# jynik/OOKiedokie

Measured on AMD Instinct MI355X. Metric: IQ Msamples/s demodulated (SC16Q11->bits), higher is better.
Workload: dtype f32

## Files before the change

### ookiedokie_amd/csrc/fir_mfma.hip

```cpp
#include "kernels.hpp"
#include "common.hpp"

#include <hip/hip_ext.h>

#include <algorithm>
#include <cmath>
#include <cstring>
#include <type_traits>

#pragma clang fp contract(off)

namespace ookd {

typedef _Float16 h8 __attribute__((ext_vector_type(8)));
typedef _Float16 h4 __attribute__((ext_vector_type(4)));
typedef float f16x __attribute__((ext_vector_type(16)));
typedef float v2fm __attribute__((ext_vector_type(2)));
typedef short v2s __attribute__((ext_vector_type(2)));
typedef uint32_t v4u __attribute__((ext_vector_type(4)));

__host__ __device__ constexpr uint32_t mslot(uint32_t j) { return j + 8u * (j >> 5); }

template <int KS, int FMT = (int)kFmtSc16>
struct MfmaGeom {
    static constexpr uint32_t Tp = 16u * (KS - 2);
    static constexpr uint32_t W = kMfmaTile + Tp;
    static constexpr uint32_t plane = mslot(W);
    static constexpr uint32_t lds_bytes = plane * 2u * 2u;
    static constexpr uint32_t vsamples = FMT == (int)kFmtSc16 ? 4u : 8u;
    static constexpr uint32_t nvec = W / vsamples;
    static constexpr int rounds = (int)((nvec + 63u) / 64u);
};

typedef const __attribute__((address_space(1))) v4u *gptr128;
__device__ __forceinline__ uint4 ld_nt4m(gptr128 p) {
    const v4u v = __builtin_nontemporal_load(p);
    return make_uint4(v.x, v.y, v.z, v.w);
}

typedef const __attribute__((address_space(1))) unsigned char *gbytes;
typedef __attribute__((address_space(1))) unsigned char *gbytes_w;
__device__ __forceinline__ uint4 ld_nt4_at(gbytes base, uint32_t byte_off) {
    const v4u v = __builtin_nontemporal_load(reinterpret_cast<gptr128>(base + byte_off));
    return make_uint4(v.x, v.y, v.z, v.w);
}

template <typename P>
__device__ __forceinline__ P uniform_ptr(P ptr) {
    uint64_t v = (uint64_t)ptr;
    asm volatile("" : "+s"(v));
    return (P)v;
}

__device__ __forceinline__ v2s as_v2sm(uint32_t w) { return __builtin_bit_cast(v2s, w); }

typedef const __attribute__((address_space(1))) uint32_t *gptr32;
typedef const __attribute__((address_space(1))) uint16_t *gptr16;
typedef const __attribute__((address_space(1))) float *gptrf;

template <int FMT>
struct RawSrcT {
    typedef typename std::conditional<FMT == (int)kFmtSc16, uint32_t, uint16_t>::type elem;
    typedef const __attribute__((address_space(1))) elem *ptr;
    ptr src;
    ptr halo;
    uint32_t halo_len;
    uint64_t n_valid;
};

typedef RawSrcT<(int)kFmtSc16> RawSrc;

template <int FMT>
__device__ __forceinline__ uint32_t fetch_fmt_m(const RawSrcT<FMT> &rs, int64_t n) {
    const uint32_t z = FMT == (int)kFmtSc16 ? 0u : zero8<FMT>();
    if (n < 0) {
        const int64_t h = (int64_t)rs.halo_len + n;
        if (h < 0 || !rs.halo) return z;
        return rs.halo[h];
    }
    if ((uint64_t)n >= rs.n_valid) return z;
    return rs.src[n];
}

template <int FMT>
__device__ __forceinline__ uint32_t fetch_raw_m(const RawSrcT<FMT> &rs, int64_t n) {
    if (n < 0) {
        const int64_t h = (int64_t)rs.halo_len + n;
        if (h < 0 || !rs.halo) return 0u;
        if constexpr (FMT == (int)kFmtSc16) return rs.halo[h];
        else return widen8<FMT>(rs.halo[h]);
    }
    if ((uint64_t)n >= rs.n_valid) return 0u;
    if constexpr (FMT == (int)kFmtSc16) return rs.src[n];
    else return widen8<FMT>(rs.src[n]);
}

template <int FMT>
__device__ __forceinline__ float2 mfma_exact_output(const RawSrcT<FMT> &rs, gptrf taps, uint32_t T, int64_t n) {
    const float s = 1.0f / 2048.0f;
    float re = 0.0f, im = 0.0f;
    for (uint32_t k = 0; k < T; ++k) {
        const uint32_t w = fetch_raw_m(rs, n - (int64_t)k);
        const float xr = (float)(int16_t)(w & 0xffffu) * s;
        const float xi = (float)(int16_t)(w >> 16) * s;
        const float t = taps[k];
        const float pr = t * xr;
        const float pi = t * xi;
        re = re + pr;
        im = im + pi;
    }
    return make_float2(re, im);
}

template <int HALF>
__device__ __forceinline__ uint32_t cvt2(uint32_t a, uint32_t b) {
    uint32_t r;
    if (HALF == 0) {
        asm("v_cvt_f16_i16_sdwa %0, %1 dst_sel:WORD_0 dst_unused:UNUSED_PAD src0_sel:WORD_0" : "=v"(r) : "v"(a));
        asm("v_cvt_f16_i16_sdwa %0, %1 dst_sel:WORD_1 dst_unused:UNUSED_PRESERVE src0_sel:WORD_0" : "+v"(r) : "v"(b));
    } else {
        asm("v_cvt_f16_i16_sdwa %0, %1 dst_sel:WORD_0 dst_unused:UNUSED_PAD src0_sel:WORD_1" : "=v"(r) : "v"(a));
        asm("v_cvt_f16_i16_sdwa %0, %1 dst_sel:WORD_1 dst_unused:UNUSED_PRESERVE src0_sel:WORD_1" : "+v"(r) : "v"(b));
    }
    return r;
}

__device__ __forceinline__ void cvt4(uint4 q, uint32_t mask, uint2 &re, uint2 &im) {
    const uint32_t w0 = q.x & mask, w1 = q.y & mask, w2 = q.z & mask, w3 = q.w & mask;
    re = make_uint2(cvt2<0>(w0, w1), cvt2<0>(w2, w3));
    im = make_uint2(cvt2<1>(w0, w1), cvt2<1>(w2, w3));
}

typedef _Float16 h2 __attribute__((ext_vector_type(2)));
typedef unsigned short v2us __attribute__((ext_vector_type(2)));

template <int FMT>
__device__ __forceinline__ void expand8(uint32_t w, uint32_t &re, uint32_t &im) {
    if (FMT == (int)kFmtCs8) w ^= 0x80808080u;
    re = __builtin_amdgcn_perm(0x64646464u, w, 0x04020400u);
    im = __builtin_amdgcn_perm(0x64646464u, w, 0x04030401u);
}

__device__ __forceinline__ uint32_t scale8(uint32_t t) {
    const h2 k = {(_Float16)16.0f, (_Float16)16.0f}, b = {(_Float16)-18432.0f, (_Float16)-18432.0f};
    return __builtin_bit_cast(uint32_t, __builtin_elementwise_fma(__builtin_bit_cast(h2, t), k, b));
}

template <int FMT>
__device__ __forceinline__ void cvt8(uint4 q, uint4 &re, uint4 &im) {
    uint32_t r0, r1, r2, r3, i0, i1, i2, i3;
    expand8<FMT>(q.x, r0, i0);
    expand8<FMT>(q.y, r1, i1);
    expand8<FMT>(q.z, r2, i2);
    expand8<FMT>(q.w, r3, i3);
    re = make_uint4(scale8(r0), scale8(r1), scale8(r2), scale8(r3));
    im = make_uint4(scale8(i0), scale8(i1), scale8(i2), scale8(i3));
}

template <int FMT, int ROUNDS>
__device__ __forceinline__ void window_levels8(const uint4 (&q)[ROUNDS], int L, bool &loud) {
    v2us mx = (v2us){0x6480, 0x6480}, mn = mx;
#pragma unroll
    for (int i = 0; i < ROUNDS; ++i) {
        const uint32_t w[4] = {q[i].x, q[i].y, q[i].z, q[i].w};
#pragma unroll
        for (int k = 0; k < 4; ++k) {
            uint32_t re, im;
            expand8<FMT>(w[k], re, im);
            const v2us a = __builtin_bit_cast(v2us, re), b = __builtin_bit_cast(v2us, im);
            mx = __builtin_elementwise_max(mx, __builtin_elementwise_max(a, b));
            mn = __builtin_elementwise_min(mn, __builtin_elementwise_min(a, b));
        }
    }
    const int m = (L - 1) >> 4;
    const uint32_t hi = 0x6480u + (uint32_t)(m < 127 ? m : 127), lo = 0x6480u - (uint32_t)(m < 128 ? m : 128);
    loud = L <= 0 || mx.x > hi || mx.y > hi || mn.x < lo || mn.y < lo;
}

template <int KS>
__host__ __device__ constexpr int mfma_waves() { return KS <= 6 ? 4 : KS <= 10 ? 8 : 16; }
constexpr uint32_t kMfmaCtlBytes = 16;

template <int KS>
__host__ __device__ constexpr uint32_t mfma_lds_bytes() {
    return (uint32_t)KS * 2u * 1024u + kMfmaCtlBytes + (uint32_t)mfma_waves<KS>() * MfmaGeom<KS>::lds_bytes;
}

template <int FMT>
struct MfmaTileCtxT {
    RawSrcT<FMT> rs;
    uint32_t *ctl;
    uint32_t tickets;
    uint64_t tile_base, tile_end;
    uint32_t xcd_span;
    bool aligned16;
};

template <int FMT>
__device__ __forceinline__ bool mfma_take_ticket(const MfmaTileCtxT<FMT> &c, uint32_t tid, uint64_t &tile) {
    uint32_t tk = 0;
    if (tid == 0) tk = __hip_atomic_fetch_add(&c.ctl[0], 1u, __ATOMIC_RELAXED, __HIP_MEMORY_SCOPE_WORKGROUP);
    tk = (uint32_t)__builtin_amdgcn_readfirstlane((int)tk);
    const uint64_t v = (uint64_t)tk * gridDim.x + blockIdx.x;
    tile = (c.xcd_span ? (v & 7u) * (uint64_t)c.xcd_span + (v >> 3) : v) + c.tile_base;
    return tk < c.tickets && v + c.tile_base < c.tile_end;
}

template <int KS, int FMT>
__device__ __forceinline__ bool mfma_interior(const MfmaTileCtxT<FMT> &c, uint64_t tile) {
    const uint64_t t0 = tile * kMfmaTile;
    return c.aligned16 && t0 >= MfmaGeom<KS>::Tp && t0 + kMfmaTile <= c.rs.n_valid;
}

template <int KS, int FMT>
__device__ __forceinline__ void mfma_issue_loads(const MfmaTileCtxT<FMT> &c, uint64_t tile, uint32_t tid,
                                                 uint4 (&q)[MfmaGeom<KS, FMT>::rounds]) {
    using Gm = MfmaGeom<KS, FMT>;
    const gbytes src4 = uniform_ptr((gbytes)(c.rs.src + (tile * kMfmaTile - Gm::Tp)));
#pragma unroll
    for (int i = 0; i < Gm::rounds; ++i) {
        const uint32_t v = tid + 64u * i;
        q[i] = ld_nt4_at(src4, 16u * ((64u * (i + 1) <= Gm::nvec || v < Gm::nvec) ? v : Gm::nvec - 1u));
    }
}

template <int FMT>
__device__ __forceinline__ uint4 fetch_vec_m(const RawSrcT<FMT> &rs, int64_t s0) {
    uint4 w;
    if constexpr (FMT == (int)kFmtSc16) {
        w.x = fetch_raw_m(rs, s0);
        w.y = fetch_raw_m(rs, s0 + 1);
        w.z = fetch_raw_m(rs, s0 + 2);
        w.w = fetch_raw_m(rs, s0 + 3);
    } else {
        w.x = fetch_fmt_m(rs, s0) | (fetch_fmt_m(rs, s0 + 1) << 16);
        w.y = fetch_fmt_m(rs, s0 + 2) | (fetch_fmt_m(rs, s0 + 3) << 16);
        w.z = fetch_fmt_m(rs, s0 + 4) | (fetch_fmt_m(rs, s0 + 5) << 16);
        w.w = fetch_fmt_m(rs, s0 + 6) | (fetch_fmt_m(rs, s0 + 7) << 16);
    }
    return w;
}

template <int KS, int FMT>
__device__ __noinline__ void mfma_boundary_stage(RawSrcT<FMT> rs, uint64_t t0, uint32_t tid, uint4 *stage) {
    using Gm = MfmaGeom<KS, FMT>;
    for (uint32_t v = tid; v < Gm::nvec; v += 64u) {
        const int64_t s0 = (int64_t)t0 - (int64_t)Gm::Tp + (int64_t)Gm::vsamples * (int64_t)v;
        stage[v] = fetch_vec_m(rs, s0);
    }
}

template <int KS, int FMT>
__device__ __forceinline__ void mfma_boundary_loads(const MfmaTileCtxT<FMT> &c, uint64_t tile, uint32_t tid, unsigned char *win,
                                                    uint4 (&q)[MfmaGeom<KS, FMT>::rounds]) {
    using Gm = MfmaGeom<KS, FMT>;
    uint4 *stage = reinterpret_cast<uint4 *>(win);
    mfma_boundary_stage<KS, FMT>(c.rs, tile * kMfmaTile, tid, stage);
    __builtin_amdgcn_fence(__ATOMIC_RELEASE, "wavefront");
    __builtin_amdgcn_wave_barrier();
    __builtin_amdgcn_fence(__ATOMIC_ACQUIRE, "wavefront");
#pragma unroll
    for (int i = 0; i < Gm::rounds; ++i) {
        const uint32_t v = tid + 64u * i;
        q[i] = stage[(64u * (i + 1) <= Gm::nvec || v < Gm::nvec) ? v : Gm::nvec - 1u];
    }
    __builtin_amdgcn_fence(__ATOMIC_RELEASE, "wavefront");
    __builtin_amdgcn_wave_barrier();
}

template <int KS, int FMT>
__device__ __forceinline__ void mfma_convert(const uint4 (&q)[MfmaGeom<KS, FMT>::rounds], uint32_t mask, uint32_t tid,
                                             _Float16 *pl_re, _Float16 *pl_im) {
    using Gm = MfmaGeom<KS, FMT>;
#pragma unroll
    for (int i = 0; i < Gm::rounds; ++i) {
        const uint32_t v = tid + 64u * i;
        if (64u * (i + 1) <= Gm::nvec || v < Gm::nvec) {
            if constexpr (FMT == (int)kFmtSc16) {
                uint2 r4, i4;
                cvt4(q[i], mask, r4, i4);
                *reinterpret_cast<uint2 *>(pl_re + mslot(4u * v)) = r4;
                *reinterpret_cast<uint2 *>(pl_im + mslot(4u * v)) = i4;
            } else {
                uint4 r8, i8;
                cvt8<FMT>(q[i], r8, i8);
                *reinterpret_cast<uint4 *>(pl_re + mslot(8u * v)) = r8;
                *reinterpret_cast<uint4 *>(pl_im + mslot(8u * v)) = i8;
            }
        }
    }
    __builtin_amdgcn_fence(__ATOMIC_RELEASE, "wavefront");
    __builtin_amdgcn_wave_barrier();
    __builtin_amdgcn_fence(__ATOMIC_ACQUIRE, "wavefront");
}

template <int KS, bool FIRST>
__device__ __forceinline__ void mfma_ksteps(const h8 *a_img, const _Float16 *pl_re, const _Float16 *pl_im, uint32_t tid,
                                            f16x &are, f16x &aim) {
    const uint32_t n = tid & 31u, hh = tid >> 5;
    const _Float16 *bre = pl_re + 40u * n + 8u * hh;
    const _Float16 *bim = pl_im + 40u * n + 8u * hh;
    const h8 *af = a_img + tid;
    f16x zero;
#pragma unroll
    for (int r = 0; r < 16; ++r) zero[r] = 0.0f;
    h8 xr = *reinterpret_cast<const h8 *>(bre), xi = *reinterpret_cast<const h8 *>(bim);
    h8 a0 = af[0], a1 = af[64];
#pragma unroll
    for (int s = 0; s < KS; ++s) {
        h8 xr_n = xr, xi_n = xi, a0_n = a0, a1_n = a1;
        if (s + 1 < KS) {
            xr_n = *reinterpret_cast<const h8 *>(bre + 16 * (s + 1) + 8 * ((s + 1) >> 1));
            xi_n = *reinterpret_cast<const h8 *>(bim + 16 * (s + 1) + 8 * ((s + 1) >> 1));
            a0_n = af[((s + 1) * 2 + 0) * 64];
            a1_n = af[((s + 1) * 2 + 1) * 64];
        }
        are = __builtin_amdgcn_mfma_f32_32x32x16_f16(a0, xr, (FIRST && s == 0) ? zero : are, 0, 0, 0);
        aim = __builtin_amdgcn_mfma_f32_32x32x16_f16(a0, xi, (FIRST && s == 0) ? zero : aim, 0, 0, 0);
        are = __builtin_amdgcn_mfma_f32_32x32x16_f16(a1, xr, are, 0, 0, 0);
        aim = __builtin_amdgcn_mfma_f32_32x32x16_f16(a1, xi, aim, 0, 0, 0);
        __builtin_amdgcn_sched_barrier(0);
        xr = xr_n;
        xi = xi_n;
        a0 = a0_n;
        a1 = a1_n;
    }
    __builtin_amdgcn_fence(__ATOMIC_RELEASE, "wavefront");
    __builtin_amdgcn_wave_barrier();
}

template <int KS>
__device__ __noinline__ void mfma_fetch_image(const void *image, unsigned char *smem, uint32_t tid) {
    v4u *dst = reinterpret_cast<v4u *>(smem) + tid;
    const gptr128 src = reinterpret_cast<gptr128>((gbytes)image) + tid;
    for (int i = 0; i < 2 * KS; i += 4) {
        const v4u f0 = src[64 * i], f1 = src[64 * i + 64], f2 = src[64 * i + 128], f3 = src[64 * i + 192];
        dst[64 * i] = f0;
        dst[64 * i + 64] = f1;
        dst[64 * i + 128] = f2;
        dst[64 * i + 192] = f3;
    }
}

template <int KS, int FMT>
__global__ __launch_bounds__(64 * mfma_waves<KS>()) __attribute__((amdgpu_waves_per_eu(4)))
void fir1_mfma_kernel(const FrontParams p) {
    constexpr int kMfmaWaves = mfma_waves<KS>();
    extern __shared__ __attribute__((aligned(16))) unsigned char smem_raw[];
    using Gm = MfmaGeom<KS, FMT>;
    typedef typename RawSrcT<FMT>::elem raw_t;
    typedef typename RawSrcT<FMT>::ptr raw_ptr;
    constexpr uint32_t kImgBytes = (uint32_t)KS * 2u * 1024u;
    uint32_t tid = threadIdx.x & 63u;
    const uint32_t wave = threadIdx.x >> 6;
    const uint32_t cap = blockIdx.y;
    MfmaTileCtxT<FMT> c;
    c.rs.src = (raw_ptr)(reinterpret_cast<const raw_t *>(p.iq) + (uint64_t)cap * p.cap_stride);
    c.rs.halo = (raw_ptr)reinterpret_cast<const raw_t *>(p.halo);
    c.rs.halo_len = p.halo_len;
    c.rs.n_valid = p.n_valid;
    c.ctl = reinterpret_cast<uint32_t *>(smem_raw + kImgBytes);
    c.tickets = p.mfma_g * (uint32_t)kMfmaWaves;
    c.tile_base = p.tile_base;
    c.tile_end = p.tile_end;
    c.xcd_span = p.mfma_xcd_span;
    c.aligned16 = (((uintptr_t)c.rs.src & 15u) == 0);
    typedef __attribute__((address_space(1))) uint64_t *gptr64;
    typedef __attribute__((address_space(1))) uint32_t *gptr32w;
    const gptr64 words = (gptr64)(p.bits + (uint64_t)cap * p.words_per_cap);
    const gptr32w tile_info = (gptr32w)(p.tile_info + (uint64_t)cap * p.tiles_per_cap);
    const h8 *a_img = reinterpret_cast<const h8 *>(smem_raw);
    unsigned char *win = smem_raw + kImgBytes + kMfmaCtlBytes + wave * Gm::lds_bytes;
    _Float16 *pl_re = reinterpret_cast<_Float16 *>(win);
    _Float16 *pl_im = pl_re + Gm::plane;
    typedef __attribute__((address_space(1))) v2fm *gptrf2;
    const gptrf2 fout = p.fir_out ? (gptrf2)(reinterpret_cast<v2fm *>(p.fir_out) + (uint64_t)cap * p.n_out) : (gptrf2)nullptr;

    if (threadIdx.x == 0) {
        c.ctl[0] = 0;
        c.ctl[1] = 0;
    }
    __syncthreads();


    uint64_t tile = 0;
    if (!mfma_take_ticket(c, tid, tile)) return;
    uint4 q[Gm::rounds];
    if (mfma_interior<KS, FMT>(c, tile)) mfma_issue_loads<KS, FMT>(c, tile, tid, q);
    else mfma_boundary_loads<KS, FMT>(c, tile, tid, win, q);
    for (;;) {
        asm volatile("" : "+v"(tid));
        const uint32_t n = tid & 31u, hh = tid >> 5;
        const uint64_t t0 = tile * kMfmaTile;
        bool loud, wide;
        if constexpr (FMT == (int)kFmtSc16) {
            v2s mx = (v2s){0, 0}, mn = (v2s){0, 0};
#pragma unroll
            for (int i = 0; i < Gm::rounds; ++i) {
                mx = __builtin_elementwise_max(mx, __builtin_elementwise_max(as_v2sm(q[i].x), as_v2sm(q[i].y)));
                mx = __builtin_elementwise_max(mx, __builtin_elementwise_max(as_v2sm(q[i].z), as_v2sm(q[i].w)));
                mn = __builtin_elementwise_min(mn, __builtin_elementwise_min(as_v2sm(q[i].x), as_v2sm(q[i].y)));
                mn = __builtin_elementwise_min(mn, __builtin_elementwise_min(as_v2sm(q[i].z), as_v2sm(q[i].w)));
            }
            const int L = p.quiet_lsb;
            loud = !(mx.x < L && mx.y < L && mn.x > -L && mn.y > -L);
            wide = __ballot(mx.x > 2047 || mx.y > 2047 || mn.x < -2048 || mn.y < -2048) != 0;
        } else {
            window_levels8<FMT>(q, p.quiet_lsb, loud);
            wide = false;
        }
        const bool quiet = (!fout && __ballot(loud) == 0) || (p.mfma_debug & 1u);

        uint64_t tile_n = 0;
        bool more = false, pre = false;
        if (quiet) {
            more = mfma_take_ticket(c, tid, tile_n);
            pre = more && mfma_interior<KS, FMT>(c, tile_n);
            if (pre) mfma_issue_loads<KS, FMT>(c, tile_n, tid, q);
            if (!p.sparse) {
                if (tid < kMfmaTile / 64) *reinterpret_cast<gptr64>(uniform_ptr((gbytes_w)(words + (t0 >> 6))) + 8u * tid) = 0;
                if (tid == 0) *uniform_ptr(tile_info + tile) = 0;
            }
            if (p.quiet_count && tid == 0) atomicAdd(p.quiet_count + ((blockIdx.x * kMfmaWaves + wave) % kQuietCounters), 1u);
        } else {
            if (__hip_atomic_load(&c.ctl[1], __ATOMIC_RELAXED, __HIP_MEMORY_SCOPE_WORKGROUP) == 0) {
                mfma_fetch_image<KS>(p.mfma_a, smem_raw, tid);
                __builtin_amdgcn_fence(__ATOMIC_RELEASE, "wavefront");
                __builtin_amdgcn_wave_barrier();
                if (tid == 0) __hip_atomic_store(&c.ctl[1], 1u, __ATOMIC_RELAXED, __HIP_MEMORY_SCOPE_WORKGROUP);
                __builtin_amdgcn_fence(__ATOMIC_ACQUIRE, "wavefront");
            }
            f16x are, aim;
            if (FMT != (int)kFmtSc16 || !wide) {
                mfma_convert<KS, FMT>(q, 0xffffffffu, tid, pl_re, pl_im);
                more = mfma_take_ticket(c, tid, tile_n);
                pre = more && mfma_interior<KS, FMT>(c, tile_n);
                if (pre) mfma_issue_loads<KS, FMT>(c, tile_n, tid, q);
                mfma_ksteps<KS, true>(a_img, pl_re, pl_im, tid, are, aim);
            } else if constexpr (FMT == (int)kFmtSc16) {
                mfma_convert<KS, FMT>(q, 0xffe0ffe0u, tid, pl_re, pl_im);
                mfma_ksteps<KS, true>(a_img, pl_re, pl_im, tid, are, aim);
                mfma_convert<KS, FMT>(q, 0x001f001fu, tid, pl_re, pl_im);
                more = mfma_take_ticket(c, tid, tile_n);
                pre = more && mfma_interior<KS, FMT>(c, tile_n);
                if (pre) mfma_issue_loads<KS, FMT>(c, tile_n, tid, q);
                mfma_ksteps<KS, false>(a_img, pl_re, pl_im, tid, are, aim);
            }

            const float plo = wide ? p.p_lo_w : p.p_lo_n;
            const float phi = wide ? p.p_hi_w : p.p_hi_n;
            const uint32_t ocol = 32u * n + 4u * hh;
            uint32_t m16 = 0;
            uint64_t any_unsure = 0;
#pragma unroll
            for (int r2 = 7; r2 >= 0; --r2) {
                const v2fm zr = (v2fm){are[2 * r2], are[2 * r2 + 1]}, zi = (v2fm){aim[2 * r2], aim[2 * r2 + 1]};
                const v2fm rr = zr * zr, ii = zi * zi;
                const v2fm pw = rr + ii;
                {
                    const uint64_t ge_hi = __ballot(pw.y >= phi);
                    asm("v_addc_co_u32_e64 %0, vcc, %0, %0, %1" : "+v"(m16) : "s"(ge_hi) : "vcc");
                    any_unsure |= __ballot(pw.y >= plo) & ~ge_hi;
                }
                {
                    const uint64_t ge_hi = __ballot(pw.x >= phi);
                    asm("v_addc_co_u32_e64 %0, vcc, %0, %0, %1" : "+v"(m16) : "s"(ge_hi) : "vcc");
                    any_unsure |= __ballot(pw.x >= plo) & ~ge_hi;
                }
            }
            if (any_unsure != 0) {
                uint32_t todo = 0, redo = 0;
#pragma unroll
                for (int r = 0; r < 16; ++r) {
                    const float rr = are[r] * are[r], ii = aim[r] * aim[r];
                    const float pw = rr + ii;
                    if (pw >= plo && !(pw >= phi)) todo |= 1u << r;
                }
                while (todo) {
                    const uint32_t r = (uint32_t)__ffs((int)todo) - 1u;
                    todo &= todo - 1u;
                    const uint64_t o = t0 + ocol + (r & 3u) + 8u * (r >> 2);
                    if (o >= p.n_out) continue;
                    const float2 y = mfma_exact_output(c.rs, (gptrf)p.taps, p.stage[0].ntaps, (int64_t)o);
                    const float rr = y.x * y.x, ii = y.y * y.y;
                    const float pe = rr + ii;
                    m16 = (m16 & ~(1u << r)) | ((pe >= p.p_star ? 1u : 0u) << r);
                    redo++;
                }
                if (redo && p.recompute_count) atomicAdd(p.recompute_count, (unsigned long long)redo);
            }
            if (fout) {
                const float cs = p.mfma_c;
#pragma unroll
                for (int r = 0; r < 16; ++r) {
                    const uint64_t o = t0 + ocol + (r & 3) + 8 * (r >> 2);
                    if (o < p.n_out) fout[o] = (v2fm){are[r] * cs, aim[r] * cs};
                }
            }

            uint32_t m32 = (m16 & 0xfu) | ((m16 & 0xf0u) << 4) | ((m16 & 0xf00u) << 8) | ((m16 & 0xf000u) << 12);
            m32 <<= 4u * hh;
            uint32_t w32 = m32 | (uint32_t)__shfl_xor((int)m32, 32);
            {
                const uint64_t c0 = t0 + 32u * n;
                if (c0 + 32u > p.n_out) {
                    const uint32_t keep = c0 >= p.n_out ? 0u : (uint32_t)(p.n_out - c0);
                    w32 &= (1u << keep) - 1u;
                }
            }
            {
                const uint32_t prev_top = (uint32_t)__shfl_up((int)(w32 >> 31), 1);
                uint32_t ch = w32 ^ (w32 << 1);
                if (n != 0) ch ^= prev_top & 1u;
                else ch &= ~1u;
                uint32_t cnt = hh == 0 ? (uint32_t)__popc(ch) : 0u;
#pragma unroll
                for (int d = 16; d >= 1; d >>= 1) cnt += (uint32_t)__shfl_xor((int)cnt, d);
                const uint32_t first = (uint32_t)__builtin_amdgcn_readfirstlane((int)(w32 & 1u));
                const uint32_t last = (uint32_t)__builtin_amdgcn_readlane((int)(w32 >> 31), 31);
                const uint64_t chl = __ballot(hh == 0 && ch != 0);
                const uint32_t widx = chl ? (uint32_t)__builtin_ctzll(chl) >> 1 : 0u;
                if (tid == 0) *uniform_ptr(tile_info + tile) = cnt | (widx << kTileWordShift) | (first << 30) | (last << 31) | p.stamp_bits;
            }
            const uint32_t up = (uint32_t)__shfl_xor((int)w32, 1);
            if (hh == 0 && (n & 1u) == 0) {
                const gbytes_w wb = uniform_ptr((gbytes_w)(words + (t0 >> 6)));
                *reinterpret_cast<gptr64>(wb + 4u * n) = (uint64_t)w32 | ((uint64_t)up << 32);
            }
        }

        if (!more) break;
        if (!pre) mfma_boundary_loads<KS, FMT>(c, tile_n, tid, win, q);
        tile = tile_n;
    }
}

constexpr uint32_t kF2Out = 256;
constexpr uint32_t kF2Tp = 96;
constexpr uint32_t kF2W = 4 * kF2Out + kF2Tp;
template <int FMT>
struct F2Geom {
    static constexpr uint32_t vsamples = FMT == (int)kFmtSc16 ? 4u : 8u;
    static constexpr uint32_t nvec = kF2W / vsamples;
    static constexpr int rounds = (int)((nvec + 63) / 64);
};
constexpr int kF2KS = 5;
constexpr int kF2Waves = 4;
__host__ __device__ constexpr uint32_t f2slot(uint32_t j) { return j + 8u * (j >> 6); }
constexpr uint32_t kF2Plane = f2slot(kF2W) + 8u;
constexpr uint32_t kF2WaveBytes = kF2Plane * 2u * 2u;
constexpr uint32_t kF2ImgBytes = kF2KS * 2u * 1024u;
constexpr uint32_t kF2LdsBytes = kF2ImgBytes + kMfmaCtlBytes + kF2Waves * kF2WaveBytes;

typedef float f4x __attribute__((ext_vector_type(4)));

struct F2Taps {
    gptrf taps1, taps2;
    uint32_t n1, n2;
};

template <int FMT>
__device__ __forceinline__ float2 fir2_mfma_exact_output(const RawSrcT<FMT> &rs, const F2Taps &ft, int64_t m) {
    const float s = 1.0f / 2048.0f;
    float re2 = 0.0f, im2 = 0.0f;
    for (uint32_t k2 = 0; k2 < ft.n2; ++k2) {
        const int64_t j1 = 2 * m + 1 - (int64_t)k2;
        float re1 = 0.0f, im1 = 0.0f;
        for (uint32_t k1 = 0; k1 < ft.n1; ++k1) {
            const uint32_t w = fetch_raw_m(rs, 2 * j1 + 1 - (int64_t)k1);
            const float xr = (float)(int16_t)(w & 0xffffu) * s;
            const float xi = (float)(int16_t)(w >> 16) * s;
            const float t = ft.taps1[k1];
            const float pr = t * xr;
            const float pi = t * xi;
            re1 = re1 + pr;
            im1 = im1 + pi;
        }
        const float t2 = ft.taps2[k2];
        const float pr = t2 * re1;
        const float pi = t2 * im1;
        re2 = re2 + pr;
        im2 = im2 + pi;
    }
    return make_float2(re2, im2);
}

template <int FMT>
__device__ __forceinline__ bool f2_interior(const MfmaTileCtxT<FMT> &c, uint64_t tile) {
    const uint64_t i0 = tile * (4ull * kF2Out);
    return c.aligned16 && i0 >= kF2Tp && i0 + 4ull * kF2Out <= c.rs.n_valid;
}

template <int FMT>
__device__ __forceinline__ void f2_issue_loads(const MfmaTileCtxT<FMT> &c, uint64_t tile, uint32_t tid,
                                               uint4 (&q)[F2Geom<FMT>::rounds]) {
    constexpr uint32_t kF2Nvec = F2Geom<FMT>::nvec;
    constexpr int kF2Rounds = F2Geom<FMT>::rounds;
    const gbytes src4 = uniform_ptr((gbytes)(c.rs.src + (tile * (4ull * kF2Out) - kF2Tp)));
#pragma unroll
    for (int i = 0; i < kF2Rounds; ++i) {
        const uint32_t v = tid + 64u * i;
        q[i] = ld_nt4_at(src4, 16u * ((64u * (i + 1) <= kF2Nvec || v < kF2Nvec) ? v : kF2Nvec - 1u));
    }
}

template <int FMT>
__device__ __noinline__ void f2_boundary_stage(RawSrcT<FMT> rs, uint64_t i0, uint32_t tid, uint4 *stage) {
    for (uint32_t v = tid; v < F2Geom<FMT>::nvec; v += 64u) {
        const int64_t s0 = (int64_t)i0 - (int64_t)kF2Tp + (int64_t)F2Geom<FMT>::vsamples * (int64_t)v;
        stage[v] = fetch_vec_m(rs, s0);
    }
}

template <int FMT>
__device__ __forceinline__ void f2_boundary_loads(const MfmaTileCtxT<FMT> &c, uint64_t tile, uint32_t tid, unsigned char *win,
                                                  uint4 (&q)[F2Geom<FMT>::rounds]) {
    constexpr uint32_t kF2Nvec = F2Geom<FMT>::nvec;
    constexpr int kF2Rounds = F2Geom<FMT>::rounds;
    uint4 *stage = reinterpret_cast<uint4 *>(win);
    f2_boundary_stage(c.rs, tile * (4ull * kF2Out), tid, stage);
    __builtin_amdgcn_fence(__ATOMIC_RELEASE, "wavefront");
    __builtin_amdgcn_wave_barrier();
    __builtin_amdgcn_fence(__ATOMIC_ACQUIRE, "wavefront");
#pragma unroll
    for (int i = 0; i < kF2Rounds; ++i) {
        const uint32_t v = tid + 64u * i;
        q[i] = stage[(64u * (i + 1) <= kF2Nvec || v < kF2Nvec) ? v : kF2Nvec - 1u];
    }
    __builtin_amdgcn_fence(__ATOMIC_RELEASE, "wavefront");
    __builtin_amdgcn_wave_barrier();
}

template <int FMT>
__device__ __forceinline__ void f2_convert(const uint4 (&q)[F2Geom<FMT>::rounds], uint32_t mask, uint32_t tid, _Float16 *pl_re,
                                           _Float16 *pl_im) {
    constexpr uint32_t kF2Nvec = F2Geom<FMT>::nvec;
    constexpr int kF2Rounds = F2Geom<FMT>::rounds;
#pragma unroll
    for (int i = 0; i < kF2Rounds; ++i) {
        const uint32_t v = tid + 64u * i;
        if (64u * (i + 1) <= kF2Nvec || v < kF2Nvec) {
            if constexpr (FMT == (int)kFmtSc16) {
                uint2 r4, i4;
                cvt4(q[i], mask, r4, i4);
                *reinterpret_cast<uint2 *>(pl_re + f2slot(4u * v)) = r4;
                *reinterpret_cast<uint2 *>(pl_im + f2slot(4u * v)) = i4;
            } else {
                uint4 r8, i8;
                cvt8<FMT>(q[i], r8, i8);
                *reinterpret_cast<uint4 *>(pl_re + f2slot(8u * v)) = r8;
                *reinterpret_cast<uint4 *>(pl_im + f2slot(8u * v)) = i8;
            }
        }
    }
    __builtin_amdgcn_fence(__ATOMIC_RELEASE, "wavefront");
    __builtin_amdgcn_wave_barrier();
    __builtin_amdgcn_fence(__ATOMIC_ACQUIRE, "wavefront");
}

template <bool FIRST>
__device__ __forceinline__ void f2_ksteps(const h8 *a_img, const _Float16 *pl_re, const _Float16 *pl_im, uint32_t tid,
                                          f4x &are, f4x &aim) {
    const uint32_t n = tid & 15u, g = tid >> 4;
    const _Float16 *bre = pl_re + 72u * n + 8u * g;
    const _Float16 *bim = pl_im + 72u * n + 8u * g;
    const h8 *af = a_img + tid;
    f4x zero = {0.0f, 0.0f, 0.0f, 0.0f};
#pragma unroll
    for (int s = 0; s < kF2KS; ++s) {
        const h8 xr = *reinterpret_cast<const h8 *>(bre + 32 * s + 8 * (s >> 1));
        const h8 xi = *reinterpret_cast<const h8 *>(bim + 32 * s + 8 * (s >> 1));
        const h8 a0 = af[(s * 2 + 0) * 64];
        const h8 a1 = af[(s * 2 + 1) * 64];
        are = __builtin_amdgcn_mfma_f32_16x16x32_f16(a0, xr, (FIRST && s == 0) ? zero : are, 0, 0, 0);
        aim = __builtin_amdgcn_mfma_f32_16x16x32_f16(a0, xi, (FIRST && s == 0) ? zero : aim, 0, 0, 0);
        are = __builtin_amdgcn_mfma_f32_16x16x32_f16(a1, xr, are, 0, 0, 0);
        aim = __builtin_amdgcn_mfma_f32_16x16x32_f16(a1, xi, aim, 0, 0, 0);
        __builtin_amdgcn_sched_barrier(0);
    }
    __builtin_amdgcn_fence(__ATOMIC_RELEASE, "wavefront");
    __builtin_amdgcn_wave_barrier();
}

__device__ __noinline__ void f2_fetch_image(const void *image, unsigned char *smem, uint32_t tid) {
    v4u *dst = reinterpret_cast<v4u *>(smem) + tid;
    const gptr128 src = reinterpret_cast<gptr128>((gbytes)image) + tid;
    for (int i = 0; i < 2 * kF2KS; i += 2) {
        const v4u f0 = src[64 * i], f1 = src[64 * i + 64];
        dst[64 * i] = f0;
        dst[64 * i + 64] = f1;
    }
}

template <int FMT>
__global__ __launch_bounds__(64 * kF2Waves) __attribute__((amdgpu_waves_per_eu(4)))
void fir2_mfma_kernel(const FrontParams p) {
    extern __shared__ __attribute__((aligned(16))) unsigned char smem_raw[];
    constexpr int kF2Rounds = F2Geom<FMT>::rounds;
    typedef typename RawSrcT<FMT>::elem raw_t;
    typedef typename RawSrcT<FMT>::ptr raw_ptr;
    uint32_t tid = threadIdx.x & 63u;
    const uint32_t wave = threadIdx.x >> 6;
    const uint32_t cap = blockIdx.y;
    MfmaTileCtxT<FMT> c;
    c.rs.src = (raw_ptr)(reinterpret_cast<const raw_t *>(p.iq) + (uint64_t)cap * p.cap_stride);
    c.rs.halo = (raw_ptr)reinterpret_cast<const raw_t *>(p.halo);
    c.rs.halo_len = p.halo_len;
    c.rs.n_valid = p.n_valid;
    c.ctl = reinterpret_cast<uint32_t *>(smem_raw + kF2ImgBytes);
    c.tickets = p.mfma_g * (uint32_t)kF2Waves;
    c.tile_base = p.tile_base;
    c.tile_end = p.tile_end;
    c.xcd_span = p.mfma_xcd_span;
    c.aligned16 = (((uintptr_t)c.rs.src & 15u) == 0);
    F2Taps ft;
    ft.taps1 = (gptrf)(p.taps + p.stage[0].tap_off);
    ft.taps2 = (gptrf)(p.taps + p.stage[1].tap_off);
    ft.n1 = p.stage[0].ntaps;
    ft.n2 = p.stage[1].ntaps;
    typedef __attribute__((address_space(1))) uint64_t *gptr64;
    typedef __attribute__((address_space(1))) uint32_t *gptr32w;
    const gptr64 words = (gptr64)(p.bits + (uint64_t)cap * p.words_per_cap);
    const gptr32w tile_info = (gptr32w)(p.tile_info + (uint64_t)cap * p.tiles_per_cap);
    const h8 *a_img = reinterpret_cast<const h8 *>(smem_raw);
    unsigned char *win = smem_raw + kF2ImgBytes + kMfmaCtlBytes + wave * kF2WaveBytes;
    _Float16 *pl_re = reinterpret_cast<_Float16 *>(win);
    _Float16 *pl_im = pl_re + kF2Plane;
    typedef __attribute__((address_space(1))) v2fm *gptrf2;
    const gptrf2 fout = p.fir_out ? (gptrf2)(reinterpret_cast<v2fm *>(p.fir_out) + (uint64_t)cap * p.n_out) : (gptrf2)nullptr;

    if (threadIdx.x == 0) {
        c.ctl[0] = 0;
        c.ctl[1] = 0;
    }
    __syncthreads();

    uint64_t tile = 0;
    if (!mfma_take_ticket(c, tid, tile)) return;
    uint4 q[kF2Rounds];
    if (f2_interior(c, tile)) f2_issue_loads(c, tile, tid, q);
    else f2_boundary_loads(c, tile, tid, win, q);
    for (;;) {
        asm volatile("" : "+v"(tid));
        const uint32_t n = tid & 15u, g = tid >> 4;
        const uint64_t M0 = tile * kF2Out;
        bool loud, wide;
        if constexpr (FMT == (int)kFmtSc16) {
            v2s mx = (v2s){0, 0}, mn = (v2s){0, 0};
#pragma unroll
            for (int i = 0; i < kF2Rounds; ++i) {
                mx = __builtin_elementwise_max(mx, __builtin_elementwise_max(as_v2sm(q[i].x), as_v2sm(q[i].y)));
                mx = __builtin_elementwise_max(mx, __builtin_elementwise_max(as_v2sm(q[i].z), as_v2sm(q[i].w)));
                mn = __builtin_elementwise_min(mn, __builtin_elementwise_min(as_v2sm(q[i].x), as_v2sm(q[i].y)));
                mn = __builtin_elementwise_min(mn, __builtin_elementwise_min(as_v2sm(q[i].z), as_v2sm(q[i].w)));
            }
            const int L = p.quiet_lsb;
            loud = !(mx.x < L && mx.y < L && mn.x > -L && mn.y > -L);
            wide = __ballot(mx.x > 2047 || mx.y > 2047 || mn.x < -2048 || mn.y < -2048) != 0;
        } else {
            window_levels8<FMT>(q, p.quiet_lsb, loud);
            wide = false;
        }
        const bool quiet = (!fout && __ballot(loud) == 0) || (p.mfma_debug & 1u);

        uint64_t tile_n = 0;
        bool more = false, pre = false;
        if (quiet) {
            more = mfma_take_ticket(c, tid, tile_n);
            pre = more && f2_interior(c, tile_n);
            if (pre) f2_issue_loads(c, tile_n, tid, q);
            if (!p.sparse) {
                if (tid < kF2Out / 64) *reinterpret_cast<gptr64>(uniform_ptr((gbytes_w)(words + (M0 >> 6))) + 8u * tid) = 0;
                if (tid == 0) *uniform_ptr(tile_info + tile) = 0;
            }
            if (p.quiet_count && tid == 0) atomicAdd(p.quiet_count + ((blockIdx.x * kF2Waves + wave) % kQuietCounters), 1u);
        } else {
            if (__hip_atomic_load(&c.ctl[1], __ATOMIC_RELAXED, __HIP_MEMORY_SCOPE_WORKGROUP) == 0) {
                f2_fetch_image(p.mfma_a, smem_raw, tid);
                __builtin_amdgcn_fence(__ATOMIC_RELEASE, "wavefront");
                __builtin_amdgcn_wave_barrier();
                if (tid == 0) __hip_atomic_store(&c.ctl[1], 1u, __ATOMIC_RELAXED, __HIP_MEMORY_SCOPE_WORKGROUP);
                __builtin_amdgcn_fence(__ATOMIC_ACQUIRE, "wavefront");
            }
            f4x are, aim;
            if (FMT != (int)kFmtSc16 || !wide) {
                f2_convert<FMT>(q, 0xffffffffu, tid, pl_re, pl_im);
                more = mfma_take_ticket(c, tid, tile_n);
                pre = more && f2_interior(c, tile_n);
                if (pre) f2_issue_loads(c, tile_n, tid, q);
                f2_ksteps<true>(a_img, pl_re, pl_im, tid, are, aim);
            } else if constexpr (FMT == (int)kFmtSc16) {
                f2_convert<FMT>(q, 0xffe0ffe0u, tid, pl_re, pl_im);
                f2_ksteps<true>(a_img, pl_re, pl_im, tid, are, aim);
                f2_convert<FMT>(q, 0x001f001fu, tid, pl_re, pl_im);
                more = mfma_take_ticket(c, tid, tile_n);
                pre = more && f2_interior(c, tile_n);
                if (pre) f2_issue_loads(c, tile_n, tid, q);
                f2_ksteps<false>(a_img, pl_re, pl_im, tid, are, aim);
            }
            const float plo = wide ? p.p_lo_w : p.p_lo_n;
            const float phi = wide ? p.p_hi_w : p.p_hi_n;
            const uint32_t o_lane = 16u * n + 4u * g;
            uint32_t nib = 0, unsure = 0;
#pragma unroll
            for (int r = 0; r < 4; ++r) {
                const float rr = are[r] * are[r], ii = aim[r] * aim[r];
                const float pw = rr + ii;
                const bool hi = pw >= phi;
                nib |= (hi ? 1u : 0u) << r;
                unsure |= ((!hi && pw >= plo) ? 1u : 0u) << r;
            }
            if (__ballot(unsure != 0) != 0) {
                uint32_t todo = unsure, redo = 0;
                while (todo) {
                    const uint32_t r = (uint32_t)__ffs((int)todo) - 1u;
                    todo &= todo - 1u;
                    const uint64_t o = M0 + o_lane + r;
                    if (o >= p.n_out) continue;
                    const float2 y = fir2_mfma_exact_output(c.rs, ft, (int64_t)o);
                    const float rr = y.x * y.x, ii = y.y * y.y;
                    const float pe = rr + ii;
                    nib = (nib & ~(1u << r)) | ((pe >= p.p_star ? 1u : 0u) << r);
                    redo++;
                }
                if (redo && p.recompute_count) atomicAdd(p.recompute_count, (unsigned long long)redo);
            }
            if (fout) {
                const float cs = p.mfma_c;
#pragma unroll
                for (int r = 0; r < 4; ++r) {
                    const uint64_t o = M0 + o_lane + r;
                    if (o < p.n_out) fout[o] = (v2fm){are[r] * cs, aim[r] * cs};
                }
            }
            if (M0 + o_lane + 4u > p.n_out) {
                const uint32_t keep = M0 + o_lane >= p.n_out ? 0u : (uint32_t)(p.n_out - (M0 + o_lane));
                nib &= (1u << keep) - 1u;
            }
            uint64_t w64 = (uint64_t)nib << (16u * (n & 3u) + 4u * g);
#pragma unroll
            for (int d = 1; d <= 32; d <<= 1) {
                if (d == 4 || d == 8) continue;
                const uint32_t lo = (uint32_t)__shfl_xor((int)(uint32_t)w64, d), hi = (uint32_t)__shfl_xor((int)(uint32_t)(w64 >> 32), d);
                w64 |= (uint64_t)lo | ((uint64_t)hi << 32);
            }
            {
                const uint32_t wq = n >> 2;
                const uint32_t top_prev = (uint32_t)__shfl((int)(uint32_t)(w64 >> 63), (int)((wq ? wq - 1u : 0u) << 2));
                uint64_t ch = w64 ^ ((w64 << 1) | (wq ? (uint64_t)(top_prev & 1u) : 0ull));
                if (wq == 0) ch &= ~1ull;
                uint32_t cnt = ((n & 3u) == 0 && g == 0) ? (uint32_t)__popcll(ch) : 0u;
#pragma unroll
                for (int d = 32; d >= 1; d >>= 1) cnt += (uint32_t)__shfl_xor((int)cnt, d);
                const uint32_t first = (uint32_t)__builtin_amdgcn_readfirstlane((int)(uint32_t)(w64 & 1ull));
                const uint32_t last = (uint32_t)__builtin_amdgcn_readlane((int)(uint32_t)(w64 >> 63), 12);
                const uint64_t chl = __ballot((n & 3u) == 0 && g == 0 && ch != 0);
                const uint32_t widx = chl ? (uint32_t)__builtin_ctzll(chl) >> 2 : 0u;
                if (tid == 0) *uniform_ptr(tile_info + tile) = cnt | (widx << kTileWordShift) | (first << 30) | (last << 31) | p.stamp_bits;
            }
            if ((n & 3u) == 0 && g == 0) {
                const gbytes_w wb = uniform_ptr((gbytes_w)(words + (M0 >> 6)));
                *reinterpret_cast<gptr64>(wb + 2u * n) = w64;
            }
        }

        if (!more) break;
        if (!pre) f2_boundary_loads(c, tile_n, tid, win, q);
        tile = tile_n;
    }
}


static uint16_t half_bits(_Float16 h) {
    uint16_t b;
    std::memcpy(&b, &h, 2);
    return b;
}

static int mfma_ksteps_for(uint32_t ntaps) {
    if (ntaps == 0) return 0;
    if (ntaps <= 32) return 4;
    if (ntaps <= 64) return 6;
    if (ntaps <= 128) return 10;
    if (ntaps <= 256) return 18;
    return 0;
}

bool mfma_prepare_taps(const float *taps, uint32_t ntaps, MfmaTaps &out) {
    out = MfmaTaps();
    const int KS = mfma_ksteps_for(ntaps);
    if (KS == 0) return false;
    double hmax = 0.0, sum_abs = 0.0;
    for (uint32_t k = 0; k < ntaps; ++k) {
        if (!std::isfinite(taps[k])) return false;
        hmax = std::max(hmax, std::fabs((double)taps[k]));
        sum_abs += std::fabs((double)taps[k]);
    }
    if (!(hmax > 0.0)) return false;
    int e = 0;
    (void)std::frexp(hmax, &e);
    const int sh = 15 - e;
    if (sh > 100 || sh < -100) return false;
    const double S = std::ldexp(1.0, sh);
    const double kMinNormal = std::ldexp(1.0, -14);
    std::vector<_Float16> p1(ntaps), p2(ntaps);
    double delta = 0.0, sum_hat = 0.0;
    for (uint32_t k = 0; k < ntaps; ++k) {
        const double hs = (double)taps[k] * S;
        _Float16 a = (_Float16)hs;
        if (std::fabs((double)a) < kMinNormal) a = (_Float16)0.0;
        const double r1 = hs - (double)a;
        _Float16 b = (_Float16)r1;
        if (std::fabs((double)b) < kMinNormal) b = (_Float16)0.0;
        const double r2 = r1 - (double)b;
        if (!std::isfinite((double)a) || !std::isfinite((double)b)) return false;
        p1[k] = a;
        p2[k] = b;
        delta += std::fabs(r2) / S;
        sum_hat += std::fabs((double)a + (double)b) / S;
    }
    const uint32_t Tp = 16u * (uint32_t)(KS - 2);
    out.ksteps = (uint32_t)KS;
    out.image.assign((size_t)KS * 2 * 64 * 8, 0);
    for (int s = 0; s < KS; ++s) {
        for (int pc = 0; pc < 2; ++pc) {
            for (uint32_t l = 0; l < 64; ++l) {
                const uint32_t r = l & 31u, hh = l >> 5;
                for (uint32_t j = 0; j < 8; ++j) {
                    const int64_t kk = 16 * s + 8 * (int64_t)hh + j;
                    const int64_t t = (int64_t)r + Tp - kk;
                    _Float16 v = (_Float16)0.0;
                    if (t >= 0 && t < (int64_t)ntaps) v = pc == 0 ? p1[t] : p2[t];
                    out.image[(((size_t)s * 2 + pc) * 64 + l) * 8 + j] = half_bits(v);
                }
            }
        }
    }
    out.c = (float)std::ldexp(1.0, -11 - sh);
    out.delta = delta;
    out.sum_abs = sum_abs;
    out.sum_hat = sum_hat;
    return true;
}

bool mfma_prepare_taps2(const float *taps1, uint32_t n1, const float *taps2, uint32_t n2, MfmaTaps &out) {
    out = MfmaTaps();
    if (n1 == 0 || n2 == 0 || n1 > 16 || n2 > 32) return false;
    const uint32_t ng = 2 * (n2 - 1) + n1;
    std::vector<double> g(ng, 0.0), gabs(ng, 0.0);
    for (uint32_t k2 = 0; k2 < n2; ++k2) {
        for (uint32_t k1 = 0; k1 < n1; ++k1) {
            if (!std::isfinite(taps1[k1]) || !std::isfinite(taps2[k2])) return false;
            g[2 * k2 + k1] += (double)taps2[k2] * (double)taps1[k1];
            gabs[2 * k2 + k1] += std::fabs((double)taps2[k2] * (double)taps1[k1]);
        }
    }
    double gmax = 0.0, sum_abs = 0.0;
    for (uint32_t t = 0; t < ng; ++t) {
        gmax = std::max(gmax, std::fabs(g[t]));
        sum_abs += gabs[t];
    }
    if (!(gmax > 0.0)) return false;
    int e = 0;
    (void)std::frexp(gmax, &e);
    const int sh = 15 - e;
    if (sh > 100 || sh < -100) return false;
    const double S = std::ldexp(1.0, sh);
    const double kMinNormal = std::ldexp(1.0, -14);
    std::vector<_Float16> p1(ng), p2(ng);
    double delta = 0.0, sum_hat = 0.0;
    for (uint32_t t = 0; t < ng; ++t) {
        const double hs = g[t] * S;
        _Float16 a = (_Float16)hs;
        if (std::fabs((double)a) < kMinNormal) a = (_Float16)0.0;
        const double r1 = hs - (double)a;
        _Float16 b = (_Float16)r1;
        if (std::fabs((double)b) < kMinNormal) b = (_Float16)0.0;
        const double r2 = r1 - (double)b;
        if (!std::isfinite((double)a) || !std::isfinite((double)b)) return false;
        p1[t] = a;
        p2[t] = b;
        delta += std::fabs(r2) / S + gabs[t] * std::ldexp(1.0, -50);
        sum_hat += std::fabs((double)a + (double)b) / S;
    }
    out.ksteps = (uint32_t)kF2KS;
    out.image.assign((size_t)kF2KS * 2 * 64 * 8, 0);
    for (int s = 0; s < kF2KS; ++s) {
        for (int pc = 0; pc < 2; ++pc) {
            for (uint32_t l = 0; l < 64; ++l) {
                const uint32_t i = l & 15u, q = l >> 4;
                for (uint32_t j = 0; j < 8; ++j) {
                    const int64_t kk = 32 * s + 8 * (int64_t)q + j;
                    const int64_t t = 4 * (int64_t)i + 99 - kk;
                    _Float16 v = (_Float16)0.0;
                    if (t >= 0 && t < (int64_t)ng) v = pc == 0 ? p1[t] : p2[t];
                    out.image[(((size_t)s * 2 + pc) * 64 + l) * 8 + j] = half_bits(v);
                }
            }
        }
    }
    out.c = (float)std::ldexp(1.0, -11 - sh);
    out.delta = delta;
    out.sum_abs = sum_abs;
    out.sum_hat = sum_hat;
    return true;
}

double mfma_error_bound2(const MfmaTaps &t, double e_ref, bool wide) {
    const double u = std::ldexp(1.0, -24);
    const double xmax = wide ? 16.0 : 1.0;
    const double chain = (double)t.ksteps * 32.0 * 2.0 * (wide ? 2.0 : 1.0);
    const double e_acc = chain * 2.0 * u * t.sum_hat;
    return 1.1 * (e_ref + (e_acc + t.delta) * xmax) + 78.0 * std::ldexp(1.0, -140);
}

double mfma_error_bound(const MfmaTaps &t, uint32_t ntaps, bool wide) {
    const double u = std::ldexp(1.0, -24);
    const double xmax = wide ? 16.0 : 1.0;
    const double chain = (double)t.ksteps * 16.0 * 2.0 * (wide ? 2.0 : 1.0);
    const double e_ref = ((double)ntaps + 1.0) * u * t.sum_abs;
    const double e_acc = chain * 2.0 * u * t.sum_hat;
    return 1.1 * (e_ref + e_acc + t.delta) * xmax + (double)ntaps * std::ldexp(1.0, -140);
}

bool mfma_scale_band(const MfmaTaps &t, float p, float &out) {
    if (std::isnan(p) || std::isinf(p) || p == 0.0f) {
        out = p;
        return true;
    }
    int e = 0;
    (void)std::frexp((double)t.c, &e);
    const double scaled = std::ldexp((double)p, -2 * (e - 1));
    const float f = (float)scaled;
    if (!std::isfinite(f) || (double)f != scaled || std::fabs(f) < 1.1754944e-38f) return false;
    out = f;
    return true;
}

bool front_uses_mfma(const FrontParams &p) {
    return p.mfma_a != nullptr && p.num_stages == 1 && p.stage[0].decim == 1 && p.origin == 0 && !p.iq_f32 &&
           mfma_ksteps_for(p.stage[0].ntaps) != 0;
}

bool front_uses_mfma2(const FrontParams &p) {
    return p.mfma_a != nullptr && p.num_stages == 2 && !p.iq_f32 && !p.halo_f32 && p.stage[0].decim == 2 &&
           p.stage[1].decim == 2 && p.stage[0].ntaps <= 16 && p.stage[1].ntaps <= 32 && p.origin % 4 == 0;
}

hipError_t launch_front_mfma2(const FrontParams &p, uint32_t num_captures, hipStream_t stream, hipEvent_t t0,
                              hipEvent_t t1, uint64_t tile_begin, uint64_t tile_count) {
    const uint64_t all = (p.n_out + kF2Out - 1) / kF2Out;
    const uint64_t b = tile_begin < all ? tile_begin : all;
    const uint64_t cnt = tile_count < all - b ? tile_count : all - b;
    if (cnt == 0) return hipSuccess;
    FrontParams pp = p;
    pp.tile_base = (uint32_t)b;
    pp.tile_end = b + cnt;
    if (pp.mfma_g == 0) pp.mfma_g = 1;
    pp.mfma_xcd_span = (p.mfma_xcd & 2u) && cnt % 8 == 0 && cnt / 8 <= 0xffffffffull ? (uint32_t)(cnt / 8) : 0u;
    const uint64_t grid = (cnt + (uint64_t)pp.mfma_g * kF2Waves - 1) / ((uint64_t)pp.mfma_g * kF2Waves);
    const void *fn = p.sample_fmt == kFmtCs8   ? reinterpret_cast<const void *>(&fir2_mfma_kernel<(int)kFmtCs8>)
                     : p.sample_fmt == kFmtCu8 ? reinterpret_cast<const void *>(&fir2_mfma_kernel<(int)kFmtCu8>)
                                               : reinterpret_cast<const void *>(&fir2_mfma_kernel<(int)kFmtSc16>);
    hipError_t e = ensure_dynamic_lds(fn, kF2LdsBytes);
    if (e != hipSuccess) return e;
    void *args[] = {&pp};
    e = hipExtLaunchKernel(fn, dim3((uint32_t)grid, num_captures), dim3(64 * kF2Waves), args, kF2LdsBytes, stream, t0, t1, 0);
    return e != hipSuccess ? e : hipGetLastError();
}

template <int KS>
static hipError_t launch_mfma_ks(FrontParams &pp, uint32_t num_captures, uint64_t grid, hipStream_t stream,
                                 hipEvent_t t0, hipEvent_t t1) {
    const void *fn = pp.sample_fmt == kFmtCs8   ? reinterpret_cast<const void *>(&fir1_mfma_kernel<KS, (int)kFmtCs8>)
                     : pp.sample_fmt == kFmtCu8 ? reinterpret_cast<const void *>(&fir1_mfma_kernel<KS, (int)kFmtCu8>)
                                                : reinterpret_cast<const void *>(&fir1_mfma_kernel<KS, (int)kFmtSc16>);
    const size_t lds = mfma_lds_bytes<KS>();
    hipError_t e = ensure_dynamic_lds(fn, lds);
    if (e != hipSuccess) return e;
    void *args[] = {&pp};
    e = hipExtLaunchKernel(fn, dim3((uint32_t)grid, num_captures), dim3(64 * mfma_waves<KS>()), args, lds, stream, t0, t1, 0);
    return e != hipSuccess ? e : hipGetLastError();
}

hipError_t launch_front_mfma(const FrontParams &p, uint32_t num_captures, hipStream_t stream, hipEvent_t t0,
                             hipEvent_t t1, uint64_t tile_begin, uint64_t tile_count) {
    const uint64_t all = (p.n_out + kFirTile - 1) / kFirTile * (kFirTile / kMfmaTile);
    const uint64_t b = tile_begin < all ? tile_begin : all;
    const uint64_t cnt = tile_count < all - b ? tile_count : all - b;
    if (cnt == 0) return hipSuccess;
    FrontParams pp = p;
    pp.tile_base = (uint32_t)b;
    pp.tile_end = b + cnt;
    if (pp.mfma_g == 0) pp.mfma_g = 1;
    pp.mfma_xcd_span = (p.mfma_xcd & 1u) && cnt % 8 == 0 && cnt / 8 <= 0xffffffffull ? (uint32_t)(cnt / 8) : 0u;
    auto grid_for = [&](int waves) { return (cnt + (uint64_t)pp.mfma_g * waves - 1) / ((uint64_t)pp.mfma_g * waves); };
    switch (mfma_ksteps_for(p.stage[0].ntaps)) {
    case 4: return launch_mfma_ks<4>(pp, num_captures, grid_for(mfma_waves<4>()), stream, t0, t1);
    case 6: return launch_mfma_ks<6>(pp, num_captures, grid_for(mfma_waves<6>()), stream, t0, t1);
    case 10: return launch_mfma_ks<10>(pp, num_captures, grid_for(mfma_waves<10>()), stream, t0, t1);
    case 18: return launch_mfma_ks<18>(pp, num_captures, grid_for(mfma_waves<18>()), stream, t0, t1);
    default: return hipErrorInvalidValue;
    }
}

}
```

Measured before the change: 1.510 million.

## Replace shuffle-based bit packing and reductions with DPP and permlane swaps

Replaces ds_bpermute-style __shfl_xor/__shfl_up reductions in the bit-packing and tile-info epilogues of both MFMA FIR kernels with DPP row shifts, permlane32/16 swaps and readlane sums. It also skips the tail-masking branch for interior tiles and simplifies LDS store addressing in the convert step by precomputing per-lane base pointers. The aim is to cut cross-lane communication latency and instruction count in the per-tile epilogue. It risks subtle lane-mapping errors, for example the changed words store width and ballot masks, and relies on gfx950-specific permlane builtins.

```diff
diff --git a/ookiedokie_amd/csrc/fir_mfma.hip b/ookiedokie_amd/csrc/fir_mfma.hip
--- a/ookiedokie_amd/csrc/fir_mfma.hip
+++ b/ookiedokie_amd/csrc/fir_mfma.hip
@@ -53,6 +53,35 @@
 }
 
 __device__ __forceinline__ v2s as_v2sm(uint32_t w) { return __builtin_bit_cast(v2s, w); }
+
+constexpr int kDppWaveShr1 = 0x138;
+constexpr int kDppRowShr = 0x110;
+template <int CTRL>
+__device__ __forceinline__ uint32_t dpp0(uint32_t x) {
+    return (uint32_t)__builtin_amdgcn_update_dpp(0, (int)x, CTRL, 0xf, 0xf, true);
+}
+
+__device__ __forceinline__ uint32_t or_halves(uint32_t x) {
+    const auto r = __builtin_amdgcn_permlane32_swap(x, x, false, false);
+    return r[0] | r[1];
+}
+
+__device__ __forceinline__ uint32_t or_row_pairs(uint32_t x) {
+    const auto r = __builtin_amdgcn_permlane16_swap(x, x, false, false);
+    return r[0] | r[1];
+}
+
+__device__ __forceinline__ uint32_t row_scan_add(uint32_t x) {
+    x += dpp0<kDppRowShr + 1>(x);
+    x += dpp0<kDppRowShr + 2>(x);
+    x += dpp0<kDppRowShr + 4>(x);
+    x += dpp0<kDppRowShr + 8>(x);
+    return x;
+}
+
+__device__ __forceinline__ uint32_t lane_value(uint32_t x, int lane) {
+    return (uint32_t)__builtin_amdgcn_readlane((int)x, lane);
+}
 
 typedef const __attribute__((address_space(1))) uint32_t *gptr32;
 typedef const __attribute__((address_space(1))) uint16_t *gptr16;
@@ -272,20 +301,25 @@
 __device__ __forceinline__ void mfma_convert(const uint4 (&q)[MfmaGeom<KS, FMT>::rounds], uint32_t mask, uint32_t tid,
                                              _Float16 *pl_re, _Float16 *pl_im) {
     using Gm = MfmaGeom<KS, FMT>;
+    _Float16 *dre = pl_re + mslot(Gm::vsamples * tid);
+    _Float16 *dim = dre + Gm::plane;
+    (void)pl_im;
 #pragma unroll
     for (int i = 0; i < Gm::rounds; ++i) {
-        const uint32_t v = tid + 64u * i;
-        if (64u * (i + 1) <= Gm::nvec || v < Gm::nvec) {
+        constexpr uint32_t kAll = 64u;
+        const uint32_t off = mslot(Gm::vsamples * 64u * (uint32_t)i);
+        const uint32_t left = Gm::nvec - 64u * (uint32_t)i;
+        if (left >= kAll || tid < left) {
             if constexpr (FMT == (int)kFmtSc16) {
                 uint2 r4, i4;
                 cvt4(q[i], mask, r4, i4);
-                *reinterpret_cast<uint2 *>(pl_re + mslot(4u * v)) = r4;
-                *reinterpret_cast<uint2 *>(pl_im + mslot(4u * v)) = i4;
+                *reinterpret_cast<uint2 *>(dre + off) = r4;
+                *reinterpret_cast<uint2 *>(dim + off) = i4;
             } else {
                 uint4 r8, i8;
                 cvt8<FMT>(q[i], r8, i8);
-                *reinterpret_cast<uint4 *>(pl_re + mslot(8u * v)) = r8;
-                *reinterpret_cast<uint4 *>(pl_im + mslot(8u * v)) = i8;
+                *reinterpret_cast<uint4 *>(dre + off) = r8;
+                *reinterpret_cast<uint4 *>(dim + off) = i8;
             }
         }
     }
@@ -500,8 +534,8 @@
 
             uint32_t m32 = (m16 & 0xfu) | ((m16 & 0xf0u) << 4) | ((m16 & 0xf00u) << 8) | ((m16 & 0xf000u) << 12);
             m32 <<= 4u * hh;
-            uint32_t w32 = m32 | (uint32_t)__shfl_xor((int)m32, 32);
-            {
+            uint32_t w32 = or_halves(m32);
+            if (t0 + kMfmaTile > p.n_out) {
                 const uint64_t c0 = t0 + 32u * n;
                 if (c0 + 32u > p.n_out) {
                     const uint32_t keep = c0 >= p.n_out ? 0u : (uint32_t)(p.n_out - c0);
@@ -509,23 +543,20 @@
                 }
             }
             {
-                const uint32_t prev_top = (uint32_t)__shfl_up((int)(w32 >> 31), 1);
-                uint32_t ch = w32 ^ (w32 << 1);
-                if (n != 0) ch ^= prev_top & 1u;
-                else ch &= ~1u;
-                uint32_t cnt = hh == 0 ? (uint32_t)__popc(ch) : 0u;
-#pragma unroll
-                for (int d = 16; d >= 1; d >>= 1) cnt += (uint32_t)__shfl_xor((int)cnt, d);
+                const uint32_t prev_top = dpp0<kDppWaveShr1>(w32 >> 31);
+                uint32_t ch = w32 ^ (w32 << 1) ^ prev_top;
+                if (n == 0) ch &= ~1u;
+                const uint32_t run = row_scan_add((uint32_t)__popc(ch));
+                const uint32_t cnt = lane_value(run, 15) + lane_value(run, 31);
                 const uint32_t first = (uint32_t)__builtin_amdgcn_readfirstlane((int)(w32 & 1u));
-                const uint32_t last = (uint32_t)__builtin_amdgcn_readlane((int)(w32 >> 31), 31);
-                const uint64_t chl = __ballot(hh == 0 && ch != 0);
-                const uint32_t widx = chl ? (uint32_t)__builtin_ctzll(chl) >> 1 : 0u;
+                const uint32_t last = lane_value(w32 >> 31, 31);
+                const uint32_t chl = (uint32_t)__ballot(ch != 0);
+                const uint32_t widx = chl ? (uint32_t)__builtin_ctz(chl) >> 1 : 0u;
                 if (tid == 0) *uniform_ptr(tile_info + tile) = cnt | (widx << kTileWordShift) | (first << 30) | (last << 31) | p.stamp_bits;
             }
-            const uint32_t up = (uint32_t)__shfl_xor((int)w32, 1);
-            if (hh == 0 && (n & 1u) == 0) {
+            if (hh == 0) {
                 const gbytes_w wb = uniform_ptr((gbytes_w)(words + (t0 >> 6)));
-                *reinterpret_cast<gptr64>(wb + 4u * n) = (uint64_t)w32 | ((uint64_t)up << 32);
+                *reinterpret_cast<gptr32w>(wb + 4u * n) = w32;
             }
         }
 
@@ -636,20 +667,25 @@
                                            _Float16 *pl_im) {
     constexpr uint32_t kF2Nvec = F2Geom<FMT>::nvec;
     constexpr int kF2Rounds = F2Geom<FMT>::rounds;
+    constexpr uint32_t kVs = F2Geom<FMT>::vsamples;
+    _Float16 *dre = pl_re + f2slot(kVs * tid);
+    _Float16 *dim = dre + kF2Plane;
+    (void)pl_im;
 #pragma unroll
     for (int i = 0; i < kF2Rounds; ++i) {
-        const uint32_t v = tid + 64u * i;
-        if (64u * (i + 1) <= kF2Nvec || v < kF2Nvec) {
+        const uint32_t off = f2slot(kVs * 64u * (uint32_t)i);
+        const uint32_t left = kF2Nvec - 64u * (uint32_t)i;
+        if (left >= 64u || tid < left) {
             if constexpr (FMT == (int)kFmtSc16) {
                 uint2 r4, i4;
                 cvt4(q[i], mask, r4, i4);
-                *reinterpret_cast<uint2 *>(pl_re + f2slot(4u * v)) = r4;
-                *reinterpret_cast<uint2 *>(pl_im + f2slot(4u * v)) = i4;
+                *reinterpret_cast<uint2 *>(dre + off) = r4;
+                *reinterpret_cast<uint2 *>(dim + off) = i4;
             } else {
                 uint4 r8, i8;
                 cvt8<FMT>(q[i], r8, i8);
-                *reinterpret_cast<uint4 *>(pl_re + f2slot(8u * v)) = r8;
-                *reinterpret_cast<uint4 *>(pl_im + f2slot(8u * v)) = i8;
+                *reinterpret_cast<uint4 *>(dre + off) = r8;
+                *reinterpret_cast<uint4 *>(dim + off) = i8;
             }
         }
     }
@@ -833,29 +869,27 @@
                     if (o < p.n_out) fout[o] = (v2fm){are[r] * cs, aim[r] * cs};
                 }
             }
-            if (M0 + o_lane + 4u > p.n_out) {
-                const uint32_t keep = M0 + o_lane >= p.n_out ? 0u : (uint32_t)(p.n_out - (M0 + o_lane));
-                nib &= (1u << keep) - 1u;
-            }
-            uint64_t w64 = (uint64_t)nib << (16u * (n & 3u) + 4u * g);
-#pragma unroll
-            for (int d = 1; d <= 32; d <<= 1) {
-                if (d == 4 || d == 8) continue;
-                const uint32_t lo = (uint32_t)__shfl_xor((int)(uint32_t)w64, d), hi = (uint32_t)__shfl_xor((int)(uint32_t)(w64 >> 32), d);
-                w64 |= (uint64_t)lo | ((uint64_t)hi << 32);
-            }
+            if (M0 + kF2Out > p.n_out) {
+                if (M0 + o_lane + 4u > p.n_out) {
+                    const uint32_t keep = M0 + o_lane >= p.n_out ? 0u : (uint32_t)(p.n_out - (M0 + o_lane));
+                    nib &= (1u << keep) - 1u;
+                }
+            }
+            const uint32_t col = or_row_pairs(or_halves(nib << (4u * g)));
+            const uint32_t lo = dpp0<0x00>(col) | (dpp0<0x55>(col) << 16);
+            const uint32_t hi = dpp0<0xaa>(col) | (dpp0<0xff>(col) << 16);
+            const uint64_t w64 = (uint64_t)lo | ((uint64_t)hi << 32);
             {
                 const uint32_t wq = n >> 2;
-                const uint32_t top_prev = (uint32_t)__shfl((int)(uint32_t)(w64 >> 63), (int)((wq ? wq - 1u : 0u) << 2));
-                uint64_t ch = w64 ^ ((w64 << 1) | (wq ? (uint64_t)(top_prev & 1u) : 0ull));
+                const uint32_t top_prev = dpp0<kDppRowShr + 4>(hi >> 31);
+                uint64_t ch = w64 ^ ((w64 << 1) | (uint64_t)top_prev);
                 if (wq == 0) ch &= ~1ull;
-                uint32_t cnt = ((n & 3u) == 0 && g == 0) ? (uint32_t)__popcll(ch) : 0u;
-#pragma unroll
-                for (int d = 32; d >= 1; d >>= 1) cnt += (uint32_t)__shfl_xor((int)cnt, d);
-                const uint32_t first = (uint32_t)__builtin_amdgcn_readfirstlane((int)(uint32_t)(w64 & 1ull));
-                const uint32_t last = (uint32_t)__builtin_amdgcn_readlane((int)(uint32_t)(w64 >> 63), 12);
-                const uint64_t chl = __ballot((n & 3u) == 0 && g == 0 && ch != 0);
-                const uint32_t widx = chl ? (uint32_t)__builtin_ctzll(chl) >> 2 : 0u;
+                const uint32_t pc = (uint32_t)__popcll(ch);
+                const uint32_t cnt = lane_value(pc, 0) + lane_value(pc, 4) + lane_value(pc, 8) + lane_value(pc, 12);
+                const uint32_t first = (uint32_t)__builtin_amdgcn_readfirstlane((int)(lo & 1u));
+                const uint32_t last = lane_value(hi >> 31, 12);
+                const uint32_t chl = (uint32_t)__ballot(ch != 0) & 0x1111u;
+                const uint32_t widx = chl ? (uint32_t)__builtin_ctz(chl) >> 2 : 0u;
                 if (tid == 0) *uniform_ptr(tile_info + tile) = cnt | (widx << kTileWordShift) | (first << 30) | (last << 31) | p.stamp_bits;
             }
             if ((n & 3u) == 0 && g == 0) {
```

Measured after the change: 1.548 million (median of 2 runs). Within noise of the previous version (+2.5%).
